# Dokumushikun/jittor-clip-fewshot

Measured on NVIDIA B200. Metric: images/sec (ViT-B/32 LoRA + MTA N=64 + LP++), higher is better.
Workload: dtype fp16

## Files before the change

### jittor-clip-fewshot_b200/csrc/gemm.cu

```cuda
#include <cstdio>
#include <mutex>
#include <unordered_map>
#include <cudaTypedefs.h>

#include "kernels.h"
#include "ptx.cuh"

namespace jcb {

namespace {

constexpr int BLOCK_M = 128;
constexpr int BLOCK_K = 64;
constexpr int UMMA_K = 16;
#ifndef JCB_GELU_WARPS
#define JCB_GELU_WARPS 4
#endif
__host__ __device__ constexpr int epi_warps_of(int epi) {
  return (epi == EPI_BIAS_GELU_BF16 || epi == EPI_LNFOLD_GELU_BF16) ? JCB_GELU_WARPS : 4;
}

#ifndef JCB_GELU_GROUP
#define JCB_GELU_GROUP 2
#endif
#ifndef JCB_GROUP
#define JCB_GROUP 2
#endif
#ifndef JCB_SMEM_KB
#define JCB_SMEM_KB 200
#endif
__host__ __device__ constexpr int group_of(int epi) { return (epi == EPI_BIAS_GELU_BF16 || epi == EPI_LNFOLD_GELU_BF16) ? JCB_GELU_GROUP : JCB_GROUP; }
__host__ __device__ constexpr bool is_lnprep(int epi) { return epi == EPI_RESID_LNPREP_SHORT || epi == EPI_RESID_LNPREP_LONG; }
__host__ __device__ constexpr bool is_lnfold(int epi) { return epi == EPI_LNFOLD_BF16 || epi == EPI_LNFOLD_GELU_BF16; }
__host__ __device__ constexpr bool out_is_bf16(int epi) { return epi == EPI_BIAS_BF16 || epi == EPI_BIAS_GELU_BF16 || is_lnfold(epi); }
#ifndef JCB_LNS_NB
#define JCB_LNS_NB 5
#endif
#ifndef JCB_LNS_D
#define JCB_LNS_D 3
#endif
#ifndef JCB_LNS_NH
#define JCB_LNS_NH 2
#endif
__host__ __device__ constexpr int lnprep_nb(int epi) { return epi == EPI_RESID_LNPREP_SHORT ? JCB_LNS_NB : 2; }
__host__ __device__ constexpr int lnprep_d(int epi) { return epi == EPI_RESID_LNPREP_SHORT ? JCB_LNS_D : 1; }
__host__ __device__ constexpr int lnprep_nh(int epi) { return epi == EPI_RESID_LNPREP_SHORT ? JCB_LNS_NH : 1; }

constexpr int CTAS = 2;

template <int BN, int EPI>
struct TileCfg {
  static constexpr int EPI_WARPS = epi_warps_of(EPI);
  static constexpr int NUM_THREADS = 64 + 32 * EPI_WARPS;
  static constexpr int HALVES = EPI_WARPS / 4;
  static constexpr int CW = BN / HALVES;
  static constexpr int GROUP = group_of(EPI) / HALVES;
  static constexpr int WARP_STAGING = (is_lnprep(EPI) ? lnprep_nb(EPI) + lnprep_nh(EPI) : GROUP) * 4096;
  static constexpr int STAGING_BYTES = EPI_WARPS * WARP_STAGING;
  static constexpr int SMEM_TOTAL = is_lnprep(EPI) ? 220 * 1024 : JCB_SMEM_KB * 1024;
  static constexpr int VEC_FLOATS = (is_lnfold(EPI) ? 2 : 1) * CW;
  static constexpr int BAR_BYTES = 512;
  static constexpr int B_ROWS = BN / CTAS;
  static constexpr int A_BYTES = BLOCK_M * BLOCK_K * 2;
  static constexpr int B_BYTES = B_ROWS * BLOCK_K * 2;
  static constexpr int STAGE_BYTES = A_BYTES + B_BYTES;
  static constexpr int STAGES = (SMEM_TOTAL - STAGING_BYTES) / STAGE_BYTES;
  static constexpr int TMEM_COLS = 2 * BN;
  static constexpr int SMEM_BYTES = STAGES * STAGE_BYTES + STAGING_BYTES + EPI_WARPS * VEC_FLOATS * 4 + BAR_BYTES + 1024;
};

struct GemmDev {
  int M, N, K;
  int K2;
  const float* bias;
  void* out;
  long long ldo;
  int* status;
  float* stats;
  int stats_slots;
  const float* colsum;
  const float* stats_in;
  const float* shift_in;
  float* shift_out;
  long long stats_in_stride;
  uint32_t idesc;
  const int* slot_of_view;
  int slot_rows;
  uint32_t slot_live;
};

__device__ __forceinline__ uint32_t tile_slot_mask(const GemmDev& p, int m_blk, int tile_m) {
  const int r0 = m_blk * tile_m;
  const int r1 = min(r0 + tile_m, p.M) - 1;
  uint32_t mask = 0;
  for (int v = r0 / p.slot_rows; v <= r1 / p.slot_rows; ++v) mask |= 1u << __ldg(p.slot_of_view + v);
  return mask & p.slot_live;
}

template <int BN, int EPI, bool F16, bool SLOTS>
__global__ void __cluster_dims__(2, 1, 1) __launch_bounds__(64 + 32 * epi_warps_of(EPI), 1)
gemm_tcgen05_2cta_kernel(const __grid_constant__ CUtensorMap tmA, const __grid_constant__ CUtensorMap tmB,
                         const __grid_constant__ CUtensorMap tmOut, const __grid_constant__ CUtensorMap tmOut2,
                         const __grid_constant__ CUtensorMap tmA2, const __grid_constant__ CUtensorMap tmB2,
                         const GemmDev p) {
  using Cfg = TileCfg<BN, EPI>;
  constexpr int STAGES = Cfg::STAGES;
  constexpr int GROUP = Cfg::GROUP;
  constexpr int WARP_STAGING = Cfg::WARP_STAGING;
  constexpr int STAGING_BYTES = Cfg::STAGING_BYTES;
  constexpr int EPI_WARPS = Cfg::EPI_WARPS;
  constexpr int CW = Cfg::CW;
  extern __shared__ uint8_t smem_raw[];
  const uint32_t raw_addr = smem_u32(smem_raw);
  uint8_t* smem = smem_raw + ((1024u - (raw_addr & 1023u)) & 1023u);
  uint8_t* ring = smem;
  uint8_t* staging = smem + STAGES * Cfg::STAGE_BYTES;
  float* s_bias_all = reinterpret_cast<float*>(staging + STAGING_BYTES);
  uint64_t* bars = reinterpret_cast<uint64_t*>(staging + STAGING_BYTES + EPI_WARPS * Cfg::VEC_FLOATS * 4);
  uint64_t* full_bar = bars;
  uint64_t* empty_bar = bars + STAGES;
  uint64_t* tmem_full_bar = bars + 2 * STAGES;
  uint64_t* tmem_empty_bar = bars + 2 * STAGES + 2;
  uint32_t* tmem_ptr_smem = reinterpret_cast<uint32_t*>(bars + 2 * STAGES + 4);
  uint64_t* load_bar = bars + 2 * STAGES + 5;

  const int warp_idx = __shfl_sync(0xffffffffu, static_cast<int>(threadIdx.x >> 5), 0);
  const int lane = threadIdx.x & 31;
  const uint32_t cta_rank = cluster_ctarank();
  const bool leader = cta_rank == 0;

  const int unit = static_cast<int>(blockIdx.x >> 1);
  const int num_units = static_cast<int>(gridDim.x >> 1);
  constexpr int TILE_M = BLOCK_M * CTAS;
  const int m_tiles = (p.M + TILE_M - 1) / TILE_M;
  const int n_tiles = p.N / BN;
  const int num_tiles = m_tiles * n_tiles;
  const int num_kb1 = p.K / BLOCK_K;
  const int num_kb = num_kb1 + p.K2 / BLOCK_K;
  constexpr uint32_t N_BLOCKS_MASK = (1u << (BN / 64)) - 1u;
  auto slot_kb_mask = [&](int m_blk) -> uint32_t { return (SLOTS && p.K2 > 0) ? tile_slot_mask(p, m_blk, TILE_M) : 0u; };
  auto slot_skip = [&](int m_blk, int n_blk) -> bool {
    return SLOTS && p.K2 == 0 && ((tile_slot_mask(p, m_blk, TILE_M) >> (n_blk * (BN / 64))) & N_BLOCKS_MASK) == 0;
  };

  if (threadIdx.x == 0) {
    tma_prefetch_desc(&tmA);
    tma_prefetch_desc(&tmB);
    if (p.K2 > 0) {
      tma_prefetch_desc(&tmA2);
      tma_prefetch_desc(&tmB2);
    }
    tma_prefetch_desc(&tmOut);
    if (is_lnprep(EPI)) {
      tma_prefetch_desc(&tmOut2);
      for (int i = 0; i < EPI_WARPS * 8; ++i) mbar_init(&load_bar[i], 1);
    }
    for (int s = 0; s < STAGES; ++s) {
      mbar_init(&full_bar[s], 1);
      mbar_init(&empty_bar[s], 1);
    }
    for (int s = 0; s < 2; ++s) {
      mbar_init(&tmem_full_bar[s], 1);
      mbar_init(&tmem_empty_bar[s], EPI_WARPS * CTAS);
    }
    fence_mbar_init();
    fence_proxy_async_smem();
  }
  if (warp_idx == 1) {
    tmem_alloc_pair(tmem_ptr_smem, Cfg::TMEM_COLS);
    tmem_relinquish_pair();
  }
  tc_fence_before();
  cluster_sync_all();
  tc_fence_after();
  const uint32_t tmem_base = *reinterpret_cast<volatile uint32_t*>(tmem_ptr_smem);
  griddep_wait();

  if (warp_idx == 0) {
    if (elect_one()) {
      int stage = 0;
      uint32_t phase = 0;
      bool ok = true;
      for (int tile = unit; tile < num_tiles && ok; tile += num_units) {
        const int m_blk = tile / n_tiles, n_blk = tile % n_tiles;
        if (slot_skip(m_blk, n_blk)) continue;
        const int m0 = m_blk * TILE_M + static_cast<int>(cta_rank) * BLOCK_M;
        const int n0 = n_blk * BN + static_cast<int>(cta_rank) * Cfg::B_ROWS;
        uint32_t kb2_rest = slot_kb_mask(m_blk);
        const int tile_kb = SLOTS && p.K2 > 0 ? num_kb1 + __popc(kb2_rest) : num_kb;
        for (int kb = 0; kb < tile_kb; ++kb) {
          if (!mbar_wait(&empty_bar[stage], phase ^ 1u, p.status, JCB_DEV_TIMEOUT_PRODUCER)) { ok = false; break; }
          uint8_t* sa = ring + stage * Cfg::STAGE_BYTES;
          uint8_t* sb = sa + Cfg::A_BYTES;
          const bool second = kb >= num_kb1;
          const CUtensorMap* ta = second ? &tmA2 : &tmA;
          const CUtensorMap* tb = second ? &tmB2 : &tmB;
          int k0 = (second ? kb - num_kb1 : kb) * BLOCK_K;
          if (SLOTS && second) {
            k0 = (__ffs(static_cast<int>(kb2_rest)) - 1) * BLOCK_K;
            kb2_rest &= kb2_rest - 1u;
          }
          if (leader) mbar_arrive_expect_tx(&full_bar[stage], 2 * Cfg::STAGE_BYTES);
          tma_load_2d_pair(sa, ta, &full_bar[stage], k0, m0);
          tma_load_2d_pair(sb, tb, &full_bar[stage], k0, n0);
          if (++stage == STAGES) { stage = 0; phase ^= 1u; }
        }
      }
    }
  } else if (warp_idx == 1) {
    if (leader && elect_one()) {
      const uint32_t idesc = p.idesc;
      int stage = 0;
      uint32_t phase = 0;
      int it = 0;
      bool ok = true;
      for (int tile = unit; tile < num_tiles && ok; tile += num_units, ++it) {
        if (slot_skip(tile / n_tiles, tile % n_tiles)) { --it; continue; }
        const int as = it & 1;
        const uint32_t aphase = (it >> 1) & 1;
        if (!mbar_wait(&tmem_empty_bar[as], aphase ^ 1u, p.status, JCB_DEV_TIMEOUT_MMA)) { ok = false; break; }
        tc_fence_after();
        const uint32_t tmem_d = tmem_base + static_cast<uint32_t>(as * BN);
        const int tile_kb = SLOTS && p.K2 > 0 ? num_kb1 + __popc(slot_kb_mask(tile / n_tiles)) : num_kb;
        for (int kb = 0; kb < tile_kb; ++kb) {
          if (!mbar_wait(&full_bar[stage], phase, p.status, JCB_DEV_TIMEOUT_MMA)) { ok = false; break; }
          tc_fence_after();
          const uint32_t sa = smem_u32(ring + stage * Cfg::STAGE_BYTES);
          const uint64_t da = umma_desc_sw128(sa);
          const uint64_t db = umma_desc_sw128(sa + Cfg::A_BYTES);
#pragma unroll
          for (int k = 0; k < BLOCK_K / UMMA_K; ++k) {
            umma_bf16_pair(tmem_d, da + static_cast<uint64_t>(2 * k), db + static_cast<uint64_t>(2 * k), idesc,
                           (kb | k) != 0 ? 1u : 0u);
          }
          umma_commit_pair(&empty_bar[stage]);
          if (++stage == STAGES) { stage = 0; phase ^= 1u; }
        }
        if (ok) umma_commit_pair(&tmem_full_bar[as]);
      }
    }
  } else {
    const int q = warp_idx & 3;
    const int ew = warp_idx - 2;
    const int col0 = (ew >> 2) * CW;
    float* s_bias = s_bias_all + ew * Cfg::VEC_FLOATS;
    float* s_csum = s_bias + CW;
    uint64_t* my_lbar = load_bar + ew * 8;
    uint32_t lphase = 0;
    const uint32_t empty_addr0 = smem_u32(&tmem_empty_bar[0]) & PEER_BIT_MASK;
    int it = 0;
    bool ok = true;
    for (int tile = unit; tile < num_tiles && ok; tile += num_units, ++it) {
      const int m_blk = tile / n_tiles, n_blk = tile % n_tiles;
      if (slot_skip(m_blk, n_blk)) { --it; continue; }
      const int as = it & 1;
      const uint32_t aphase = (it >> 1) & 1;
      __syncwarp();
      for (int i = lane; i < CW; i += 32) {
        s_bias[i] = p.bias ? __ldg(p.bias + n_blk * BN + col0 + i) : 0.0f;
        if (is_lnfold(EPI)) s_csum[i] = __ldg(p.colsum + n_blk * BN + col0 + i);
      }
      __syncwarp();
      const int row0e = m_blk * TILE_M + static_cast<int>(cta_rank) * BLOCK_M + q * 32;
      float shift = 0.f;
      if (is_lnprep(EPI)) {
        if (p.shift_in != nullptr && row0e + lane < p.M) {
          const long long r = static_cast<long long>(row0e + lane) * p.stats_in_stride;
          const float2* st = reinterpret_cast<const float2*>(p.stats_in) + r * p.stats_slots;
          float su = 0.f;
          for (int i = 0; i < p.stats_slots; ++i) su += __ldg(st + i).x;
          shift = __ldg(p.shift_in + r) + su / static_cast<float>(p.N);
        }
        if (lane == 0) {
          bulk_wait_read<0>();
#pragma unroll
          for (int d = 0; d < lnprep_d(EPI); ++d) {
            mbar_arrive_expect_tx(&my_lbar[d], 4096);
            tma_load_2d(staging + ew * WARP_STAGING + d * 4096, &tmOut, &my_lbar[d], n_blk * BN + d * 32, row0e);
          }
        }
        __syncwarp();
      }

      ok = mbar_wait(&tmem_full_bar[as], aphase, p.status, JCB_DEV_TIMEOUT_EPILOGUE);
      ok = __all_sync(0xffffffffu, ok);
      if (!ok) break;
      tc_fence_after();

      const int row0 = m_blk * TILE_M + static_cast<int>(cta_rank) * BLOCK_M + q * 32;
      const uint32_t taddr = tmem_base + (static_cast<uint32_t>(q * 32) << 16) + static_cast<uint32_t>(as * BN + col0);
      if (is_lnprep(EPI)) {
        constexpr int NB = lnprep_nb(EPI), D = lnprep_d(EPI), NH = lnprep_nh(EPI);
        constexpr int NCH = BN / 32;
        uint8_t* my_stage = staging + ew * WARP_STAGING;
        uint8_t* my_half = my_stage + NB * 4096;
        uint32_t v[2][32];
        tmem_ld_32x32b_x32(taddr, v[0]);
        float rs = 0.f, rq = 0.f;
#pragma unroll
        for (int c = 0; c < NCH; ++c) {
          uint32_t(&cur)[32] = v[c & 1];
          constexpr int WAITN = NB - D - 1;
          if (c >= 1) {
            if (lane == 0) bulk_wait_read<WAITN>();
            __syncwarp();
          }
          if (c + D < NCH && lane == 0) {
            const int nb = (c + D) % NB;
            mbar_arrive_expect_tx(&my_lbar[nb], 4096);
            tma_load_2d(my_stage + nb * 4096, &tmOut, &my_lbar[nb], n_blk * BN + (c + D) * 32, row0);
          }
          float bb[32];
#pragma unroll
          for (int j = 0; j < 8; ++j) {
            const float4 b4 = *reinterpret_cast<const float4*>(s_bias + c * 32 + 4 * j);
            bb[4 * j] = b4.x; bb[4 * j + 1] = b4.y; bb[4 * j + 2] = b4.z; bb[4 * j + 3] = b4.w;
          }
          tmem_ld_wait();
          if (c + 1 < NCH) {
            tmem_ld_32x32b_x32(taddr + static_cast<uint32_t>((c + 1) * 32), v[(c + 1) & 1]);
          } else {
            tc_fence_before();
            __syncwarp();
            if (lane == 0) mbar_arrive_cluster(empty_addr0 + static_cast<uint32_t>(as * 8));
          }
          const int b = c % NB;
          ok = mbar_wait(&my_lbar[b], (lphase >> b) & 1u, p.status, JCB_DEV_TIMEOUT_EPILOGUE);
          lphase ^= 1u << b;
          uint8_t* rowp = my_stage + b * 4096 + lane * 128;
          uint8_t* halfp = my_half + ((c >> 1) % NH) * 4096 + lane * 128;
#pragma unroll
          for (int jj = 0; jj < 4; ++jj) {
            float f[8];
#pragma unroll
            for (int h = 0; h < 2; ++h) {
              const int j = 2 * jj + h;
              float4* piece = reinterpret_cast<float4*>(rowp + ((j ^ (lane & 7)) << 4));
              float4 o = *piece;
              o.x += __uint_as_float(cur[4 * j + 0]) + bb[4 * j + 0];
              o.y += __uint_as_float(cur[4 * j + 1]) + bb[4 * j + 1];
              o.z += __uint_as_float(cur[4 * j + 2]) + bb[4 * j + 2];
              o.w += __uint_as_float(cur[4 * j + 3]) + bb[4 * j + 3];
              *piece = o;
              f[4 * h + 0] = o.x; f[4 * h + 1] = o.y; f[4 * h + 2] = o.z; f[4 * h + 3] = o.w;
            }
#pragma unroll
            for (int e = 0; e < 8; ++e) { f[e] -= shift; rs += f[e]; rq = fmaf(f[e], f[e], rq); }
            uint4 hb;
            hb.x = pack_h2<F16>(f[0], f[1]); hb.y = pack_h2<F16>(f[2], f[3]);
            hb.z = pack_h2<F16>(f[4], f[5]); hb.w = pack_h2<F16>(f[6], f[7]);
            const int hp = (c & 1) * 4 + jj;
            *reinterpret_cast<uint4*>(halfp + ((hp ^ (lane & 7)) << 4)) = hb;
          }
          fence_proxy_async_smem();
          __syncwarp();
          if (lane == 0) {
            tma_store_2d(&tmOut, my_stage + b * 4096, n_blk * BN + c * 32, row0);
            if (c & 1) tma_store_2d(&tmOut2, my_half + ((c >> 1) % NH) * 4096, n_blk * BN + (c - 1) * 32, row0);
            bulk_commit();
          }
        }
        ok = __all_sync(0xffffffffu, ok);
        if (row0 + lane < p.M) {
          *reinterpret_cast<float2*>(p.stats + (static_cast<long long>(row0 + lane) * p.stats_slots + n_blk) * 2) =
              make_float2(rs, rq);
          if (n_blk == 0 && p.shift_out != nullptr) p.shift_out[row0 + lane] = shift;
        }
      } else {
        constexpr bool OUT_BF16 = out_is_bf16(EPI);
        constexpr bool FOLD = is_lnfold(EPI);
        constexpr bool GELU = EPI == EPI_BIAS_GELU_BF16 || EPI == EPI_LNFOLD_GELU_BF16;
        constexpr int CHUNK_COLS = OUT_BF16 ? 64 : 32;
        constexpr int NCH = CW / CHUNK_COLS;
        uint8_t* my_stage = staging + ew * WARP_STAGING;
        float ln_r = 1.f, ln_nmr = 0.f;
        if (FOLD) {
          float su = 0.f, sq = 0.f;
          if (row0 + lane < p.M) {
            const float2* st = reinterpret_cast<const float2*>(p.stats) + static_cast<long long>(row0 + lane) * p.stats_slots;
            for (int i = 0; i < p.stats_slots; ++i) { const float2 t2 = __ldg(st + i); su += t2.x; sq += t2.y; }
          }
          const float inv_k = 1.0f / static_cast<float>(p.K);
          const float mean = su * inv_k;
          const float var = fmaxf(fmaf(sq, inv_k, -mean * mean), 0.f);
          ln_r = 1.0f / sqrtf(var + 1e-5f);
          ln_nmr = -mean * ln_r;
        }
        int row_slot = -1;
        if (SLOTS && p.K2 == 0 && row0 + lane < p.M) row_slot = __ldg(p.slot_of_view + (row0 + lane) / p.slot_rows);
        const int blk0 = (n_blk * BN + col0) / 64;
        (void)row_slot; (void)blk0;
        const uint64_t r2 = f2_pack(ln_r, ln_r), nmr2 = f2_pack(ln_nmr, ln_nmr);
        const uint64_t k05 = f2_pack(0.5f, 0.5f), k851 = f2_pack(0.851f, 0.851f);
        (void)r2; (void)nmr2; (void)k05; (void)k851;
        uint32_t v[2][CHUNK_COLS];
        auto load_chunk = [&](int c, uint32_t (&dst)[CHUNK_COLS]) {
          tmem_ld_32x32b_x32(taddr + static_cast<uint32_t>(c * CHUNK_COLS), *reinterpret_cast<uint32_t(*)[32]>(&dst[0]));
          if (OUT_BF16)
            tmem_ld_32x32b_x32(taddr + static_cast<uint32_t>(c * CHUNK_COLS + 32),
                               *reinterpret_cast<uint32_t(*)[32]>(&dst[CHUNK_COLS - 32]));
        };
        load_chunk(0, v[0]);
#pragma unroll
        for (int c = 0; c < NCH; ++c) {
          uint32_t(&cur)[CHUNK_COLS] = v[c & 1];
          uint64_t bb2[CHUNK_COLS / 2];
#pragma unroll
          for (int j = 0; j < CHUNK_COLS / 4; ++j) {
            const float4 b4 = *reinterpret_cast<const float4*>(s_bias + c * CHUNK_COLS + 4 * j);
            bb2[2 * j] = f2_pack(b4.x, b4.y);
            bb2[2 * j + 1] = f2_pack(b4.z, b4.w);
            if (FOLD) {
              const float4 s4 = *reinterpret_cast<const float4*>(s_csum + c * CHUNK_COLS + 4 * j);
              bb2[2 * j] = f2_fma(nmr2, f2_pack(s4.x, s4.y), bb2[2 * j]);
              bb2[2 * j + 1] = f2_fma(nmr2, f2_pack(s4.z, s4.w), bb2[2 * j + 1]);
            }
          }
          if (c % GROUP == 0) {
            if (lane == 0) bulk_wait_read<0>();
            __syncwarp();
          }
          tmem_ld_wait();
          if (c + 1 < NCH) {
            load_chunk(c + 1, v[(c + 1) & 1]);
          } else {
            tc_fence_before();
            __syncwarp();
            if (lane == 0) mbar_arrive_cluster(empty_addr0 + static_cast<uint32_t>(as * 8));
          }
          uint8_t* rowp = my_stage + (c % GROUP) * 4096 + lane * 128;
#pragma unroll
          for (int j = 0; j < 8; ++j) {
            uint4 o;
            if (OUT_BF16) {
              float f[8];
#pragma unroll
              for (int e = 0; e < 4; ++e) {
                const uint64_t a2 = f2_pack(__uint_as_float(cur[8 * j + 2 * e]), __uint_as_float(cur[8 * j + 2 * e + 1]));
                uint64_t x2 = FOLD ? f2_fma(a2, r2, bb2[4 * j + e]) : f2_add(a2, bb2[4 * j + e]);
                if (GELU) {
                  const uint64_t h2 = f2_mul(x2, k05);
                  float t0, t1;
                  f2_unpack(f2_mul(x2, k851), t0, t1);
                  x2 = f2_fma(h2, f2_pack(tanh_approx(t0), tanh_approx(t1)), h2);
                }
                f2_unpack(x2, f[2 * e], f[2 * e + 1]);
              }
              o.x = pack_h2<F16>(f[0], f[1]); o.y = pack_h2<F16>(f[2], f[3]);
              o.z = pack_h2<F16>(f[4], f[5]); o.w = pack_h2<F16>(f[6], f[7]);
              if (SLOTS && p.K2 == 0 && row_slot != blk0 + c) o = make_uint4(0u, 0u, 0u, 0u);
            } else {
              float f0, f1, f2, f3;
              f2_unpack(f2_add(f2_pack(__uint_as_float(cur[4 * j + 0]), __uint_as_float(cur[4 * j + 1])), bb2[2 * j]), f0, f1);
              f2_unpack(f2_add(f2_pack(__uint_as_float(cur[4 * j + 2]), __uint_as_float(cur[4 * j + 3])), bb2[2 * j + 1]), f2, f3);
              o.x = __float_as_uint(f0); o.y = __float_as_uint(f1); o.z = __float_as_uint(f2); o.w = __float_as_uint(f3);
            }
            *reinterpret_cast<uint4*>(rowp + ((j ^ (lane & 7)) << 4)) = o;
          }
          if (c % GROUP == GROUP - 1 || c == NCH - 1) {
            fence_proxy_async_smem();
            __syncwarp();
            if (lane == 0) {
              constexpr int G0 = 0;
#pragma unroll
              for (int g = c - (c % GROUP); g <= c; ++g) {
                const uint8_t* src = my_stage + (g % GROUP) * 4096;
                if (EPI == EPI_BIAS_RESID_F32) tma_reduce_add_2d(&tmOut, src, n_blk * BN + col0 + g * CHUNK_COLS, row0);
                else tma_store_2d(&tmOut, src, n_blk * BN + col0 + g * CHUNK_COLS, row0);
              }
              (void)G0;
              bulk_commit();
            }
          }
        }
      }
    }
    if (lane == 0) bulk_wait<0>();
  }

  tc_fence_before();
  cluster_sync_all();
  if (warp_idx == 1) {
    tc_fence_after();
    tmem_dealloc_pair(tmem_base, Cfg::TMEM_COLS);
  }
}

PFN_cuTensorMapEncodeTiled_v12000 g_encode_tiled = nullptr;
char g_driver_err[256] = {0};

struct TmapKey {
  const void* base; uint64_t rows, cols, ld; uint32_t box_rows, box_cols; int dtype;
  bool operator==(const TmapKey& o) const {
    return base == o.base && rows == o.rows && cols == o.cols && ld == o.ld && box_rows == o.box_rows &&
           box_cols == o.box_cols && dtype == o.dtype;
  }
};
struct TmapKeyHash {
  size_t operator()(const TmapKey& k) const {
    uint64_t h = reinterpret_cast<uintptr_t>(k.base) * 0x9E3779B97F4A7C15ull;
    h ^= (k.rows + 0x9E3779B97F4A7C15ull + (h << 6) + (h >> 2));
    h ^= (k.cols * 1315423911ull + k.ld * 2654435761ull + (h << 6) + (h >> 2));
    h ^= (static_cast<uint64_t>(k.box_rows) << 40) ^ (static_cast<uint64_t>(k.box_cols) << 20) ^ static_cast<uint64_t>(k.dtype);
    return static_cast<size_t>(h);
  }
};
std::mutex g_tmap_mu;
std::unordered_map<TmapKey, CUtensorMap, TmapKeyHash> g_tmap_cache;
uint64_t g_tmap_hits = 0, g_tmap_misses = 0;

bool make_tmap_2d(CUtensorMap* tm, int dtype, const void* base, uint64_t rows, uint64_t cols, uint64_t ld_elems,
                  uint32_t box_rows, uint32_t box_cols) {
  const TmapKey key{base, rows, cols, ld_elems, box_rows, box_cols, dtype};
  {
    std::lock_guard<std::mutex> lock(g_tmap_mu);
    auto it = g_tmap_cache.find(key);
    if (it != g_tmap_cache.end()) { *tm = it->second; ++g_tmap_hits; return true; }
  }
  const uint64_t esz = dtype == TM_F32 ? 4 : 2;
  cuuint64_t gdim[2] = {cols, rows};
  cuuint64_t gstride[1] = {ld_elems * esz};
  cuuint32_t box[2] = {box_cols, box_rows};
  cuuint32_t estr[2] = {1, 1};
  const CUtensorMapDataType dt = dtype == TM_F32 ? CU_TENSOR_MAP_DATA_TYPE_FLOAT32
                                 : dtype == TM_F16 ? CU_TENSOR_MAP_DATA_TYPE_FLOAT16 : CU_TENSOR_MAP_DATA_TYPE_BFLOAT16;
  CUresult r = g_encode_tiled(tm, dt, 2, const_cast<void*>(base), gdim, gstride, box, estr, CU_TENSOR_MAP_INTERLEAVE_NONE,
                              CU_TENSOR_MAP_SWIZZLE_128B, CU_TENSOR_MAP_L2_PROMOTION_L2_256B,
                              CU_TENSOR_MAP_FLOAT_OOB_FILL_NONE);
  if (r != CUDA_SUCCESS) return false;
  std::lock_guard<std::mutex> lock(g_tmap_mu);
  if (g_tmap_cache.size() >= 8192) g_tmap_cache.clear();
  g_tmap_cache.emplace(key, *tm);
  ++g_tmap_misses;
  return true;
}

template <int BN, int EPI, bool F16, bool SLOTS = false>
cudaError_t launch_cfg(const GemmArgs& a, int* dev_status, int num_sms, cudaStream_t stream) {
  using Cfg = TileCfg<BN, EPI>;
  const int op_dt = a.f16 ? TM_F16 : TM_BF16;
  CUtensorMap tmA, tmB, tmOut;
  if (!make_tmap_2d(&tmA, op_dt, a.A, a.M, a.K, a.lda, BLOCK_M, BLOCK_K)) return cudaErrorInvalidValue;
  if (!make_tmap_2d(&tmB, op_dt, a.B, a.N, a.K, a.ldb, Cfg::B_ROWS, BLOCK_K)) return cudaErrorInvalidValue;
  constexpr bool OUT_BF16 = out_is_bf16(EPI);
  CUtensorMap tmOut2;
  if (!make_tmap_2d(&tmOut, OUT_BF16 ? op_dt : TM_F32, a.out, a.M, a.N, a.ldo, 32, OUT_BF16 ? 64 : 32)) return cudaErrorInvalidValue;
  tmOut2 = tmOut;
  if (is_lnprep(EPI)) {
    if (!a.out2 || !a.stats || a.stats_slots < a.N / BN) return cudaErrorInvalidValue;
    if ((a.shift_in != nullptr) != (a.stats_in != nullptr) || a.stats_in == a.stats) return cudaErrorInvalidValue;
    if (!make_tmap_2d(&tmOut2, op_dt, a.out2, a.M, a.N, a.ldo2, 32, 64)) return cudaErrorInvalidValue;
  }
  if (is_lnfold(EPI) && (!a.stats || !a.colsum || a.stats_slots < 1)) return cudaErrorInvalidValue;
  CUtensorMap tmA2 = tmA, tmB2 = tmB;
  if (a.K2 > 0) {
    if (!make_tmap_2d(&tmA2, op_dt, a.A2, a.M, a.K2, a.lda2, BLOCK_M, BLOCK_K)) return cudaErrorInvalidValue;
    if (!make_tmap_2d(&tmB2, op_dt, a.B2, a.N, a.K2, a.ldb2, Cfg::B_ROWS, BLOCK_K)) return cudaErrorInvalidValue;
  }
  auto kern = gemm_tcgen05_2cta_kernel<BN, EPI, F16, SLOTS>;
  {
// ... 91 lines not shown
```

### jittor-clip-fewshot_b200/csrc/ptx.cuh

```cuda
#pragma once
#include <cstdint>
#include <cuda.h>
#include <cuda_bf16.h>
#include <cuda_fp16.h>
#include <cuda_runtime.h>

namespace jcb {

enum : int {
  JCB_DEV_OK = 0,
  JCB_DEV_TIMEOUT_PRODUCER = 101,
  JCB_DEV_TIMEOUT_MMA = 102,
  JCB_DEV_TIMEOUT_EPILOGUE = 103,
  JCB_DEV_SMEM_ALIGN = 104,
};

__device__ __forceinline__ uint32_t smem_u32(const void* p) {
  return static_cast<uint32_t>(__cvta_generic_to_shared(p));
}
__device__ __forceinline__ uint64_t globaltimer_ns() {
  uint64_t t;
  asm volatile("mov.u64 %0, %%globaltimer;" : "=l"(t));
  return t;
}
__device__ __forceinline__ bool elect_one() {
  uint32_t pred;
  asm volatile(
      "{\n\t.reg .pred p;\n\t"
      "elect.sync _|p, 0xffffffff;\n\t"
      "selp.u32 %0, 1, 0, p;\n\t}"
      : "=r"(pred));
  return pred != 0;
}

__device__ __forceinline__ void mbar_init(uint64_t* bar, uint32_t count) {
  asm volatile("mbarrier.init.shared::cta.b64 [%0], %1;" ::"r"(smem_u32(bar)), "r"(count) : "memory");
}
__device__ __forceinline__ void fence_mbar_init() {
  asm volatile("fence.mbarrier_init.release.cluster;" ::: "memory");
}
__device__ __forceinline__ void fence_proxy_async_smem() {
  asm volatile("fence.proxy.async.shared::cta;" ::: "memory");
}
__device__ __forceinline__ void mbar_arrive_expect_tx(uint64_t* bar, uint32_t bytes) {
  asm volatile("mbarrier.arrive.expect_tx.shared::cta.b64 _, [%0], %1;" ::"r"(smem_u32(bar)), "r"(bytes)
               : "memory");
}
__device__ __forceinline__ void mbar_arrive(uint64_t* bar) {
  asm volatile("mbarrier.arrive.shared::cta.b64 _, [%0];" ::"r"(smem_u32(bar)) : "memory");
}
__device__ __forceinline__ bool mbar_try_wait(uint64_t* bar, uint32_t parity) {
  uint32_t ok;
  asm volatile(
      "{\n\t.reg .pred p;\n\t"
      "mbarrier.try_wait.parity.shared::cta.b64 p, [%1], %2;\n\t"
      "selp.u32 %0, 1, 0, p;\n\t}"
      : "=r"(ok)
      : "r"(smem_u32(bar)), "r"(parity)
      : "memory");
  return ok != 0;
}
#ifndef JCB_MBAR_TIMEOUT_NS
#define JCB_MBAR_TIMEOUT_NS 2000000000ull
#endif
__device__ __forceinline__ bool mbar_wait(uint64_t* bar, uint32_t parity, int* status, int code) {
  if (mbar_try_wait(bar, parity)) return true;
  const uint64_t t0 = globaltimer_ns();
  uint32_t spins = 0;
  while (!mbar_try_wait(bar, parity)) {
    if (((++spins) & 255u) == 0u) {
      if (*reinterpret_cast<volatile int*>(status) != 0) return false;
      if (globaltimer_ns() - t0 > JCB_MBAR_TIMEOUT_NS) {
        atomicCAS(status, 0, code);
        return false;
      }
    }
  }
  return true;
}

__device__ __forceinline__ void tma_prefetch_desc(const CUtensorMap* tm) {
  asm volatile("prefetch.tensormap [%0];" ::"l"(reinterpret_cast<uint64_t>(tm)) : "memory");
}
__device__ __forceinline__ void tma_load_2d(void* smem_dst, const CUtensorMap* tm, uint64_t* bar, int c0,
                                            int c1) {
  asm volatile(
      "cp.async.bulk.tensor.2d.shared::cluster.global.mbarrier::complete_tx::bytes [%0], [%1, {%3, %4}], [%2];"
      ::"r"(smem_u32(smem_dst)), "l"(reinterpret_cast<uint64_t>(tm)), "r"(smem_u32(bar)), "r"(c0), "r"(c1)
      : "memory");
}


__device__ __forceinline__ void tma_store_2d(const CUtensorMap* tm, const void* smem_src, int c0, int c1) {
  asm volatile("cp.async.bulk.tensor.2d.global.shared::cta.bulk_group [%0, {%2, %3}], [%1];" ::"l"(
                   reinterpret_cast<uint64_t>(tm)),
               "r"(smem_u32(smem_src)), "r"(c0), "r"(c1)
               : "memory");
}
__device__ __forceinline__ void tma_reduce_add_2d(const CUtensorMap* tm, const void* smem_src, int c0, int c1) {
  asm volatile("cp.reduce.async.bulk.tensor.2d.global.shared::cta.add.bulk_group [%0, {%2, %3}], [%1];" ::"l"(
                   reinterpret_cast<uint64_t>(tm)),
               "r"(smem_u32(smem_src)), "r"(c0), "r"(c1)
               : "memory");
}
__device__ __forceinline__ void bulk_commit() { asm volatile("cp.async.bulk.commit_group;" ::: "memory"); }
template <int N>
__device__ __forceinline__ void bulk_wait_read() {
  asm volatile("cp.async.bulk.wait_group.read %0;" ::"n"(N) : "memory");
}
template <int N>
__device__ __forceinline__ void bulk_wait() {
  asm volatile("cp.async.bulk.wait_group %0;" ::"n"(N) : "memory");
}
__device__ __forceinline__ float tanh_approx(float x) {
  float y;
  asm("tanh.approx.f32 %0, %1;" : "=f"(y) : "f"(x));
  return y;
}

__device__ __forceinline__ void tmem_alloc(uint32_t* dst_smem, uint32_t ncols) {
  asm volatile("tcgen05.alloc.cta_group::1.sync.aligned.shared::cta.b32 [%0], %1;" ::"r"(smem_u32(dst_smem)),
               "r"(ncols)
               : "memory");
}
__device__ __forceinline__ void tmem_relinquish() {
  asm volatile("tcgen05.relinquish_alloc_permit.cta_group::1.sync.aligned;" ::: "memory");
}
__device__ __forceinline__ void tmem_dealloc(uint32_t taddr, uint32_t ncols) {
  asm volatile("tcgen05.dealloc.cta_group::1.sync.aligned.b32 %0, %1;" ::"r"(taddr), "r"(ncols) : "memory");
}
__device__ __forceinline__ void tc_fence_before() {
  asm volatile("tcgen05.fence::before_thread_sync;" ::: "memory");
}
__device__ __forceinline__ void tc_fence_after() {
  asm volatile("tcgen05.fence::after_thread_sync;" ::: "memory");
}
__device__ __forceinline__ void umma_commit(uint64_t* bar) {
  asm volatile("tcgen05.commit.cta_group::1.mbarrier::arrive::one.shared::cluster.b64 [%0];" ::"r"(
                   smem_u32(bar))
               : "memory");
}
__device__ __forceinline__ uint64_t umma_desc_sw128(uint32_t smem_addr) {
  uint64_t d = 0;
  d |= static_cast<uint64_t>((smem_addr & 0x3FFFFu) >> 4);
  d |= static_cast<uint64_t>(1) << 16;
  d |= static_cast<uint64_t>(1024 >> 4) << 32;
  d |= static_cast<uint64_t>(1) << 46;
  d |= static_cast<uint64_t>(2) << 61;
  return d;
}
__host__ __device__ constexpr uint32_t umma_idesc_bf16_f32(int m, int n) {
  return (1u << 4) | (1u << 7) | (1u << 10) | (static_cast<uint32_t>(n >> 3) << 17) |
         (static_cast<uint32_t>(m >> 4) << 24);
}
__host__ __device__ constexpr uint32_t umma_idesc_f32acc(bool f16, int m, int n, bool b_mn_major = false) {
  return (1u << 4) | (f16 ? 0u : ((1u << 7) | (1u << 10))) | (b_mn_major ? (1u << 16) : 0u) |
         (static_cast<uint32_t>(n >> 3) << 17) | (static_cast<uint32_t>(m >> 4) << 24);
}
__device__ __forceinline__ void umma_bf16(uint32_t tmem_d, uint64_t desc_a, uint64_t desc_b, uint32_t idesc,
                                          uint32_t accumulate) {
  asm volatile(
      "{\n\t.reg .pred p;\n\t"
      "setp.ne.b32 p, %4, 0;\n\t"
      "tcgen05.mma.cta_group::1.kind::f16 [%0], %1, %2, %3, p;\n\t}"
      ::"r"(tmem_d), "l"(desc_a), "l"(desc_b), "r"(idesc), "r"(accumulate)
      : "memory");
}
__device__ __forceinline__ void tmem_ld_32x32b_x32(uint32_t taddr, uint32_t (&v)[32]) {
  asm volatile(
      "tcgen05.ld.sync.aligned.32x32b.x32.b32 "
      "{%0, %1, %2, %3, %4, %5, %6, %7, %8, %9, %10, %11, %12, %13, %14, %15, "
      "%16, %17, %18, %19, %20, %21, %22, %23, %24, %25, %26, %27, %28, %29, %30, %31}, [%32];"
      : "=r"(v[0]), "=r"(v[1]), "=r"(v[2]), "=r"(v[3]), "=r"(v[4]), "=r"(v[5]), "=r"(v[6]), "=r"(v[7]),
        "=r"(v[8]), "=r"(v[9]), "=r"(v[10]), "=r"(v[11]), "=r"(v[12]), "=r"(v[13]), "=r"(v[14]), "=r"(v[15]),
        "=r"(v[16]), "=r"(v[17]), "=r"(v[18]), "=r"(v[19]), "=r"(v[20]), "=r"(v[21]), "=r"(v[22]),
// ... 184 lines not shown
```

Measured before the change: 1552.

## Add dedicated TMA loader warp for residual LN-prep epilogue loads

For the short LN-prep epilogue, the kernel gains an extra warp that issues all residual-tile TMA loads into a per-warp ring of buffers. Free/full mbarriers coordinate it with the epilogue warps, which no longer issue their own loads. Bias now comes from global memory via __ldg instead of being staged in shared memory. Optional L2 evict-first cache hints are added but off by default. The goal is to take load issue and wait latency off the epilogue critical path, at the cost of an extra warp, more barriers and per-element bias loads.

```diff
diff --git a/jittor-clip-fewshot_b200/csrc/gemm.cu b/jittor-clip-fewshot_b200/csrc/gemm.cu
--- a/jittor-clip-fewshot_b200/csrc/gemm.cu
+++ b/jittor-clip-fewshot_b200/csrc/gemm.cu
@@ -36,30 +36,34 @@
 #ifndef JCB_LNS_NB
 #define JCB_LNS_NB 5
 #endif
-#ifndef JCB_LNS_D
-#define JCB_LNS_D 3
+#ifndef JCB_LNS_K
+#define JCB_LNS_K 1
 #endif
-#ifndef JCB_LNS_NH
-#define JCB_LNS_NH 2
+#ifndef JCB_LNS_HINT
+#define JCB_LNS_HINT 0
 #endif
-__host__ __device__ constexpr int lnprep_nb(int epi) { return epi == EPI_RESID_LNPREP_SHORT ? JCB_LNS_NB : 2; }
-__host__ __device__ constexpr int lnprep_d(int epi) { return epi == EPI_RESID_LNPREP_SHORT ? JCB_LNS_D : 1; }
-__host__ __device__ constexpr int lnprep_nh(int epi) { return epi == EPI_RESID_LNPREP_SHORT ? JCB_LNS_NH : 1; }
+#ifndef JCB_LNS_SMEM_KB
+#define JCB_LNS_SMEM_KB 220
+#endif
+__host__ __device__ constexpr bool has_loader(int epi) { return epi == EPI_RESID_LNPREP_SHORT; }
+__host__ __device__ constexpr int lnprep_nb(int epi) { return has_loader(epi) ? JCB_LNS_NB : 2; }
+__host__ __device__ constexpr int lnprep_nh(int epi) { return has_loader(epi) ? 2 : 1; }
+__host__ __device__ constexpr int num_threads_of(int epi) { return 64 + 32 * epi_warps_of(epi) + (has_loader(epi) ? 32 : 0); }
 
 constexpr int CTAS = 2;
 
 template <int BN, int EPI>
 struct TileCfg {
   static constexpr int EPI_WARPS = epi_warps_of(EPI);
-  static constexpr int NUM_THREADS = 64 + 32 * EPI_WARPS;
+  static constexpr int NUM_THREADS = num_threads_of(EPI);
   static constexpr int HALVES = EPI_WARPS / 4;
   static constexpr int CW = BN / HALVES;
   static constexpr int GROUP = group_of(EPI) / HALVES;
   static constexpr int WARP_STAGING = (is_lnprep(EPI) ? lnprep_nb(EPI) + lnprep_nh(EPI) : GROUP) * 4096;
   static constexpr int STAGING_BYTES = EPI_WARPS * WARP_STAGING;
-  static constexpr int SMEM_TOTAL = is_lnprep(EPI) ? 220 * 1024 : JCB_SMEM_KB * 1024;
-  static constexpr int VEC_FLOATS = (is_lnfold(EPI) ? 2 : 1) * CW;
-  static constexpr int BAR_BYTES = 512;
+  static constexpr int SMEM_TOTAL = has_loader(EPI) ? JCB_LNS_SMEM_KB * 1024 : is_lnprep(EPI) ? 220 * 1024 : JCB_SMEM_KB * 1024;
+  static constexpr int VEC_FLOATS = has_loader(EPI) ? 0 : (is_lnfold(EPI) ? 2 : 1) * CW;
+  static constexpr int BAR_BYTES = has_loader(EPI) ? 1024 : 512;
   static constexpr int B_ROWS = BN / CTAS;
   static constexpr int A_BYTES = BLOCK_M * BLOCK_K * 2;
   static constexpr int B_BYTES = B_ROWS * BLOCK_K * 2;
@@ -98,7 +102,7 @@
 }
 
 template <int BN, int EPI, bool F16, bool SLOTS>
-__global__ void __cluster_dims__(2, 1, 1) __launch_bounds__(64 + 32 * epi_warps_of(EPI), 1)
+__global__ void __cluster_dims__(2, 1, 1) __launch_bounds__(num_threads_of(EPI), 1)
 gemm_tcgen05_2cta_kernel(const __grid_constant__ CUtensorMap tmA, const __grid_constant__ CUtensorMap tmB,
                          const __grid_constant__ CUtensorMap tmOut, const __grid_constant__ CUtensorMap tmOut2,
                          const __grid_constant__ CUtensorMap tmA2, const __grid_constant__ CUtensorMap tmB2,
@@ -123,6 +127,13 @@
   uint64_t* tmem_empty_bar = bars + 2 * STAGES + 2;
   uint32_t* tmem_ptr_smem = reinterpret_cast<uint32_t*>(bars + 2 * STAGES + 4);
   uint64_t* load_bar = bars + 2 * STAGES + 5;
+  uint64_t* free_bar = load_bar + EPI_WARPS * 8;
+  constexpr bool LOADER = has_loader(EPI);
+  constexpr int NB = lnprep_nb(EPI);
+  static_assert(!LOADER || (EPI_WARPS == 4 && NB <= 8 && JCB_LNS_K >= 0 && NB > JCB_LNS_K + 1 &&
+                            JCB_LNS_K <= 2 * lnprep_nh(EPI) - 2 && (BN / 32) % (2 * lnprep_nh(EPI)) == 0),
+                "loader ring: a buffer per chunk in flight, bf16 buffers reused in the same order in every tile");
+  static_assert(Cfg::BAR_BYTES >= (2 * STAGES + 5 + (LOADER ? 2 : 1) * EPI_WARPS * 8) * 8, "barrier region");
 
   const int warp_idx = __shfl_sync(0xffffffffu, static_cast<int>(threadIdx.x >> 5), 0);
   const int lane = threadIdx.x & 31;
@@ -154,6 +165,8 @@
     if (is_lnprep(EPI)) {
       tma_prefetch_desc(&tmOut2);
       for (int i = 0; i < EPI_WARPS * 8; ++i) mbar_init(&load_bar[i], 1);
+      if (LOADER)
+        for (int i = 0; i < EPI_WARPS * 8; ++i) mbar_init(&free_bar[i], 1);
     }
     for (int s = 0; s < STAGES; ++s) {
       mbar_init(&full_bar[s], 1);
@@ -239,7 +252,7 @@
         if (ok) umma_commit_pair(&tmem_full_bar[as]);
       }
     }
-  } else {
+  } else if (warp_idx < 2 + EPI_WARPS) {
     const int q = warp_idx & 3;
     const int ew = warp_idx - 2;
     const int col0 = (ew >> 2) * CW;
@@ -247,6 +260,9 @@
     float* s_csum = s_bias + CW;
     uint64_t* my_lbar = load_bar + ew * 8;
     uint32_t lphase = 0;
+    int rbuf = 0;
+    uint32_t rphase = 0;
+    int rfree = 0, rdone = 0;
     const uint32_t empty_addr0 = smem_u32(&tmem_empty_bar[0]) & PEER_BIT_MASK;
     int it = 0;
     bool ok = true;
@@ -256,7 +272,7 @@
       const int as = it & 1;
       const uint32_t aphase = (it >> 1) & 1;
       __syncwarp();
-      for (int i = lane; i < CW; i += 32) {
+      for (int i = lane; i < (LOADER ? 0 : CW); i += 32) {
         s_bias[i] = p.bias ? __ldg(p.bias + n_blk * BN + col0 + i) : 0.0f;
         if (is_lnfold(EPI)) s_csum[i] = __ldg(p.colsum + n_blk * BN + col0 + i);
       }
@@ -271,15 +287,14 @@
           for (int i = 0; i < p.stats_slots; ++i) su += __ldg(st + i).x;
           shift = __ldg(p.shift_in + r) + su / static_cast<float>(p.N);
         }
-        if (lane == 0) {
-          bulk_wait_read<0>();
-#pragma unroll
-          for (int d = 0; d < lnprep_d(EPI); ++d) {
-            mbar_arrive_expect_tx(&my_lbar[d], 4096);
-            tma_load_2d(staging + ew * WARP_STAGING + d * 4096, &tmOut, &my_lbar[d], n_blk * BN + d * 32, row0e);
-          }
-        }
-        __syncwarp();
+        if (!LOADER) {
+          if (lane == 0) {
+            bulk_wait_read<0>();
+            mbar_arrive_expect_tx(&my_lbar[0], 4096);
+            tma_load_2d(staging + ew * WARP_STAGING, &tmOut, &my_lbar[0], n_blk * BN, row0e);
+          }
+          __syncwarp();
+        }
       }
 
       ok = mbar_wait(&tmem_full_bar[as], aphase, p.status, JCB_DEV_TIMEOUT_EPILOGUE);
@@ -290,7 +305,7 @@
       const int row0 = m_blk * TILE_M + static_cast<int>(cta_rank) * BLOCK_M + q * 32;
       const uint32_t taddr = tmem_base + (static_cast<uint32_t>(q * 32) << 16) + static_cast<uint32_t>(as * BN + col0);
       if (is_lnprep(EPI)) {
-        constexpr int NB = lnprep_nb(EPI), D = lnprep_d(EPI), NH = lnprep_nh(EPI);
+        constexpr int D = 1, NH = lnprep_nh(EPI);
         constexpr int NCH = BN / 32;
         uint8_t* my_stage = staging + ew * WARP_STAGING;
         uint8_t* my_half = my_stage + NB * 4096;
@@ -300,21 +315,38 @@
 #pragma unroll
         for (int c = 0; c < NCH; ++c) {
           uint32_t(&cur)[32] = v[c & 1];
-          constexpr int WAITN = NB - D - 1;
-          if (c >= 1) {
-            if (lane == 0) bulk_wait_read<WAITN>();
+          if (LOADER) {
+            if (lane == 0) {
+              bulk_wait_read<JCB_LNS_K>();
+              if (rdone > JCB_LNS_K) {
+                mbar_arrive(&free_bar[ew * 8 + rfree]);
+                if (++rfree == NB) rfree = 0;
+              }
+            }
             __syncwarp();
-          }
-          if (c + D < NCH && lane == 0) {
-            const int nb = (c + D) % NB;
-            mbar_arrive_expect_tx(&my_lbar[nb], 4096);
-            tma_load_2d(my_stage + nb * 4096, &tmOut, &my_lbar[nb], n_blk * BN + (c + D) * 32, row0);
+            ++rdone;
+          } else {
+            constexpr int WAITN = NB - D - 1;
+            if (c >= 1) {
+              if (lane == 0) bulk_wait_read<WAITN>();
+              __syncwarp();
+            }
+            if (c + D < NCH && lane == 0) {
+              const int nb = (c + D) % NB;
+              mbar_arrive_expect_tx(&my_lbar[nb], 4096);
+              tma_load_2d(my_stage + nb * 4096, &tmOut, &my_lbar[nb], n_blk * BN + (c + D) * 32, row0);
+            }
           }
           float bb[32];
 #pragma unroll
           for (int j = 0; j < 8; ++j) {
-            const float4 b4 = *reinterpret_cast<const float4*>(s_bias + c * 32 + 4 * j);
-            bb[4 * j] = b4.x; bb[4 * j + 1] = b4.y; bb[4 * j + 2] = b4.z; bb[4 * j + 3] = b4.w;
+            if (LOADER) {
+#pragma unroll
+              for (int e = 0; e < 4; ++e) bb[4 * j + e] = p.bias ? __ldg(p.bias + n_blk * BN + c * 32 + 4 * j + e) : 0.0f;
+            } else {
+              const float4 b4 = *reinterpret_cast<const float4*>(s_bias + c * 32 + 4 * j);
+              bb[4 * j] = b4.x; bb[4 * j + 1] = b4.y; bb[4 * j + 2] = b4.z; bb[4 * j + 3] = b4.w;
+            }
           }
           tmem_ld_wait();
           if (c + 1 < NCH) {
@@ -324,9 +356,13 @@
             __syncwarp();
             if (lane == 0) mbar_arrive_cluster(empty_addr0 + static_cast<uint32_t>(as * 8));
           }
-          const int b = c % NB;
-          ok = mbar_wait(&my_lbar[b], (lphase >> b) & 1u, p.status, JCB_DEV_TIMEOUT_EPILOGUE);
-          lphase ^= 1u << b;
+          const int b = LOADER ? rbuf : c % NB;
+          ok = mbar_wait(&my_lbar[b], LOADER ? rphase : (lphase >> b) & 1u, p.status, JCB_DEV_TIMEOUT_EPILOGUE);
+          if (LOADER) {
+            if (++rbuf == NB) { rbuf = 0; rphase ^= 1u; }
+          } else {
+            lphase ^= 1u << b;
+          }
           uint8_t* rowp = my_stage + b * 4096 + lane * 128;
           uint8_t* halfp = my_half + ((c >> 1) % NH) * 4096 + lane * 128;
 #pragma unroll
@@ -355,7 +391,8 @@
           fence_proxy_async_smem();
           __syncwarp();
           if (lane == 0) {
-            tma_store_2d(&tmOut, my_stage + b * 4096, n_blk * BN + c * 32, row0);
+            if (LOADER && JCB_LNS_HINT) tma_store_2d_hint(&tmOut, my_stage + b * 4096, n_blk * BN + c * 32, row0, l2_evict_first_policy());
+            else tma_store_2d(&tmOut, my_stage + b * 4096, n_blk * BN + c * 32, row0);
             if (c & 1) tma_store_2d(&tmOut2, my_half + ((c >> 1) % NH) * 4096, n_blk * BN + (c - 1) * 32, row0);
             bulk_commit();
           }
@@ -476,6 +513,29 @@
       }
     }
     if (lane == 0) bulk_wait<0>();
+  } else if (LOADER) {
+    if (elect_one()) {
+      int buf = 0;
+      uint32_t phase = 0;
+      bool ok = true;
+      for (int tile = unit; tile < num_tiles && ok; tile += num_units) {
+        const int m_blk = tile / n_tiles, n_blk = tile % n_tiles;
+        const int row0c = m_blk * TILE_M + static_cast<int>(cta_rank) * BLOCK_M;
+        for (int c = 0; c < BN / 32 && ok; ++c) {
+          for (int ew = 0; ew < EPI_WARPS; ++ew) {
+            if (!mbar_wait(&free_bar[ew * 8 + buf], phase ^ 1u, p.status, JCB_DEV_TIMEOUT_PRODUCER)) { ok = false; break; }
+            mbar_arrive_expect_tx(&load_bar[ew * 8 + buf], 4096);
+            if (JCB_LNS_HINT)
+              tma_load_2d_hint(staging + ew * WARP_STAGING + buf * 4096, &tmOut, &load_bar[ew * 8 + buf], n_blk * BN + c * 32,
+                               row0c + ((ew + 2) & 3) * 32, l2_evict_first_policy());
+            else
+              tma_load_2d(staging + ew * WARP_STAGING + buf * 4096, &tmOut, &load_bar[ew * 8 + buf], n_blk * BN + c * 32,
+                          row0c + ((ew + 2) & 3) * 32);
+          }
+          if (++buf == NB) { buf = 0; phase ^= 1u; }
+        }
+      }
+    }
   }
 
   tc_fence_before();
diff --git a/jittor-clip-fewshot_b200/csrc/ptx.cuh b/jittor-clip-fewshot_b200/csrc/ptx.cuh
--- a/jittor-clip-fewshot_b200/csrc/ptx.cuh
+++ b/jittor-clip-fewshot_b200/csrc/ptx.cuh
@@ -89,8 +89,25 @@
       ::"r"(smem_u32(smem_dst)), "l"(reinterpret_cast<uint64_t>(tm)), "r"(smem_u32(bar)), "r"(c0), "r"(c1)
       : "memory");
 }
-
-
+__device__ __forceinline__ uint64_t l2_evict_first_policy() {
+  uint64_t pol;
+  asm volatile("createpolicy.fractional.L2::evict_first.b64 %0, 1.0;" : "=l"(pol));
+  return pol;
+}
+__device__ __forceinline__ void tma_load_2d_hint(void* smem_dst, const CUtensorMap* tm, uint64_t* bar, int c0, int c1,
+                                                 uint64_t policy) {
+  asm volatile(
+      "cp.async.bulk.tensor.2d.shared::cluster.global.mbarrier::complete_tx::bytes.L2::cache_hint [%0], [%1, {%3, %4}], [%2], %5;"
+      ::"r"(smem_u32(smem_dst)), "l"(reinterpret_cast<uint64_t>(tm)), "r"(smem_u32(bar)), "r"(c0), "r"(c1), "l"(policy)
+      : "memory");
+}
+
+__device__ __forceinline__ void tma_store_2d_hint(const CUtensorMap* tm, const void* smem_src, int c0, int c1, uint64_t policy) {
+  asm volatile("cp.async.bulk.tensor.2d.global.shared::cta.bulk_group.L2::cache_hint [%0, {%2, %3}], [%1], %4;" ::"l"(
+                   reinterpret_cast<uint64_t>(tm)),
+               "r"(smem_u32(smem_src)), "r"(c0), "r"(c1), "l"(policy)
+               : "memory");
+}
 __device__ __forceinline__ void tma_store_2d(const CUtensorMap* tm, const void* smem_src, int c0, int c1) {
   asm volatile("cp.async.bulk.tensor.2d.global.shared::cta.bulk_group [%0, {%2, %3}], [%1];" ::"l"(
                    reinterpret_cast<uint64_t>(tm)),
```

Result: no change. 1547, median of 6 (-0.3%).

## Add dedicated residual-load producer warp for LNPREP epilogue with full/empty ring

Applied to the files above, without the earlier changes.

Moves residual tile TMA loads in the LNPREP epilogue from each epilogue warp's lane 0 into a new dedicated producer warp. The producer and consumers coordinate through per-warp full/empty mbarrier rings, so loads can run ahead across tiles instead of being prefetched only within a tile. The bias is now read directly from global memory instead of being staged in shared memory, which frees space for more pipeline stages. The cost is an extra warp per CTA and a more complex barrier protocol, with buffers released after a lagged bulk_wait_read.

```diff
diff --git a/jittor-clip-fewshot_b200/csrc/gemm.cu b/jittor-clip-fewshot_b200/csrc/gemm.cu
--- a/jittor-clip-fewshot_b200/csrc/gemm.cu
+++ b/jittor-clip-fewshot_b200/csrc/gemm.cu
@@ -34,39 +34,44 @@
 __host__ __device__ constexpr bool is_lnfold(int epi) { return epi == EPI_LNFOLD_BF16 || epi == EPI_LNFOLD_GELU_BF16; }
 __host__ __device__ constexpr bool out_is_bf16(int epi) { return epi == EPI_BIAS_BF16 || epi == EPI_BIAS_GELU_BF16 || is_lnfold(epi); }
 #ifndef JCB_LNS_NB
-#define JCB_LNS_NB 5
-#endif
-#ifndef JCB_LNS_D
-#define JCB_LNS_D 3
+#define JCB_LNS_NB 4
 #endif
 #ifndef JCB_LNS_NH
 #define JCB_LNS_NH 2
 #endif
 __host__ __device__ constexpr int lnprep_nb(int epi) { return epi == EPI_RESID_LNPREP_SHORT ? JCB_LNS_NB : 2; }
-__host__ __device__ constexpr int lnprep_d(int epi) { return epi == EPI_RESID_LNPREP_SHORT ? JCB_LNS_D : 1; }
 __host__ __device__ constexpr int lnprep_nh(int epi) { return epi == EPI_RESID_LNPREP_SHORT ? JCB_LNS_NH : 1; }
+#ifndef JCB_LNS_LAG
+#define JCB_LNS_LAG 1
+#endif
+__host__ __device__ constexpr int lnprep_lag(int epi) { return epi == EPI_RESID_LNPREP_SHORT ? JCB_LNS_LAG : 0; }
+__host__ __device__ constexpr int threads_of(int epi) { return 64 + 32 * epi_warps_of(epi) + (is_lnprep(epi) ? 32 : 0); }
 
 constexpr int CTAS = 2;
 
 template <int BN, int EPI>
 struct TileCfg {
   static constexpr int EPI_WARPS = epi_warps_of(EPI);
-  static constexpr int NUM_THREADS = 64 + 32 * EPI_WARPS;
+  static constexpr int NUM_THREADS = threads_of(EPI);
   static constexpr int HALVES = EPI_WARPS / 4;
   static constexpr int CW = BN / HALVES;
   static constexpr int GROUP = group_of(EPI) / HALVES;
   static constexpr int WARP_STAGING = (is_lnprep(EPI) ? lnprep_nb(EPI) + lnprep_nh(EPI) : GROUP) * 4096;
   static constexpr int STAGING_BYTES = EPI_WARPS * WARP_STAGING;
-  static constexpr int SMEM_TOTAL = is_lnprep(EPI) ? 220 * 1024 : JCB_SMEM_KB * 1024;
-  static constexpr int VEC_FLOATS = (is_lnfold(EPI) ? 2 : 1) * CW;
-  static constexpr int BAR_BYTES = 512;
+  static constexpr int SMEM_TOTAL = is_lnprep(EPI) ? 224 * 1024 : JCB_SMEM_KB * 1024;
+  static constexpr int VEC_FLOATS = is_lnprep(EPI) ? 0 : (is_lnfold(EPI) ? 2 : 1) * CW;
   static constexpr int B_ROWS = BN / CTAS;
   static constexpr int A_BYTES = BLOCK_M * BLOCK_K * 2;
   static constexpr int B_BYTES = B_ROWS * BLOCK_K * 2;
   static constexpr int STAGE_BYTES = A_BYTES + B_BYTES;
   static constexpr int STAGES = (SMEM_TOTAL - STAGING_BYTES) / STAGE_BYTES;
+  static constexpr int BAR_BYTES = is_lnprep(EPI) ? 8 * (2 * STAGES + 5 + 2 * EPI_WARPS * lnprep_nb(EPI)) : 512;
   static constexpr int TMEM_COLS = 2 * BN;
   static constexpr int SMEM_BYTES = STAGES * STAGE_BYTES + STAGING_BYTES + EPI_WARPS * VEC_FLOATS * 4 + BAR_BYTES + 1024;
+  static_assert(SMEM_BYTES <= 227 * 1024 && STAGES >= 2, "shared memory split");
+  static_assert(!is_lnprep(EPI) || (EPI_WARPS == 4 && lnprep_nh(EPI) >= 1 && lnprep_lag(EPI) >= 0 &&
+                                    lnprep_lag(EPI) <= 2 * lnprep_nh(EPI) - 2 && lnprep_lag(EPI) < lnprep_nb(EPI)),
+                "LNPREP ring: one warp per TMEM lane quarter, a freed buffer must precede the chunk waiting for it");
 };
 
 struct GemmDev {
@@ -98,7 +103,7 @@
 }
 
 template <int BN, int EPI, bool F16, bool SLOTS>
-__global__ void __cluster_dims__(2, 1, 1) __launch_bounds__(64 + 32 * epi_warps_of(EPI), 1)
+__global__ void __cluster_dims__(2, 1, 1) __launch_bounds__(threads_of(EPI), 1)
 gemm_tcgen05_2cta_kernel(const __grid_constant__ CUtensorMap tmA, const __grid_constant__ CUtensorMap tmB,
                          const __grid_constant__ CUtensorMap tmOut, const __grid_constant__ CUtensorMap tmOut2,
                          const __grid_constant__ CUtensorMap tmA2, const __grid_constant__ CUtensorMap tmB2,
@@ -122,7 +127,9 @@
   uint64_t* tmem_full_bar = bars + 2 * STAGES;
   uint64_t* tmem_empty_bar = bars + 2 * STAGES + 2;
   uint32_t* tmem_ptr_smem = reinterpret_cast<uint32_t*>(bars + 2 * STAGES + 4);
-  uint64_t* load_bar = bars + 2 * STAGES + 5;
+  constexpr int NB = lnprep_nb(EPI);
+  uint64_t* res_full = bars + 2 * STAGES + 5;
+  uint64_t* res_empty = res_full + EPI_WARPS * NB;
 
   const int warp_idx = __shfl_sync(0xffffffffu, static_cast<int>(threadIdx.x >> 5), 0);
   const int lane = threadIdx.x & 31;
@@ -153,7 +160,10 @@
     tma_prefetch_desc(&tmOut);
     if (is_lnprep(EPI)) {
       tma_prefetch_desc(&tmOut2);
-      for (int i = 0; i < EPI_WARPS * 8; ++i) mbar_init(&load_bar[i], 1);
+      for (int i = 0; i < EPI_WARPS * NB; ++i) {
+        mbar_init(&res_full[i], 1);
+        mbar_init(&res_empty[i], 1);
+      }
     }
     for (int s = 0; s < STAGES; ++s) {
       mbar_init(&full_bar[s], 1);
@@ -239,14 +249,31 @@
         if (ok) umma_commit_pair(&tmem_full_bar[as]);
       }
     }
+  } else if (is_lnprep(EPI) && warp_idx >= 2 + EPI_WARPS) {
+    if (elect_one()) {
+      constexpr int NCH = BN / 32;
+      int g = 0;
+      bool ok = true;
+      for (int tile = unit; tile < num_tiles && ok; tile += num_units) {
+        const int m_blk = tile / n_tiles, n_blk = tile % n_tiles;
+        if (slot_skip(m_blk, n_blk)) continue;
+        for (int c = 0; c < NCH && ok; ++c, ++g) {
+          const int b = g % NB;
+          for (int ew = 0; ew < EPI_WARPS; ++ew) {
+            if (!mbar_wait(&res_empty[ew * NB + b], ((g / NB) & 1) ^ 1u, p.status, JCB_DEV_TIMEOUT_PRODUCER)) { ok = false; break; }
+            const int row0 = m_blk * TILE_M + static_cast<int>(cta_rank) * BLOCK_M + ((ew + 2) & 3) * 32;
+            mbar_arrive_expect_tx(&res_full[ew * NB + b], 4096);
+            tma_load_2d(staging + ew * WARP_STAGING + b * 4096, &tmOut, &res_full[ew * NB + b], n_blk * BN + c * 32, row0);
+          }
+        }
+      }
+    }
   } else {
     const int q = warp_idx & 3;
     const int ew = warp_idx - 2;
     const int col0 = (ew >> 2) * CW;
     float* s_bias = s_bias_all + ew * Cfg::VEC_FLOATS;
     float* s_csum = s_bias + CW;
-    uint64_t* my_lbar = load_bar + ew * 8;
-    uint32_t lphase = 0;
     const uint32_t empty_addr0 = smem_u32(&tmem_empty_bar[0]) & PEER_BIT_MASK;
     int it = 0;
     bool ok = true;
@@ -256,7 +283,7 @@
       const int as = it & 1;
       const uint32_t aphase = (it >> 1) & 1;
       __syncwarp();
-      for (int i = lane; i < CW; i += 32) {
+      for (int i = lane; i < (is_lnprep(EPI) ? 0 : CW); i += 32) {
         s_bias[i] = p.bias ? __ldg(p.bias + n_blk * BN + col0 + i) : 0.0f;
         if (is_lnfold(EPI)) s_csum[i] = __ldg(p.colsum + n_blk * BN + col0 + i);
       }
@@ -271,15 +298,6 @@
           for (int i = 0; i < p.stats_slots; ++i) su += __ldg(st + i).x;
           shift = __ldg(p.shift_in + r) + su / static_cast<float>(p.N);
         }
-        if (lane == 0) {
-          bulk_wait_read<0>();
-#pragma unroll
-          for (int d = 0; d < lnprep_d(EPI); ++d) {
-            mbar_arrive_expect_tx(&my_lbar[d], 4096);
-            tma_load_2d(staging + ew * WARP_STAGING + d * 4096, &tmOut, &my_lbar[d], n_blk * BN + d * 32, row0e);
-          }
-        }
-        __syncwarp();
       }
 
       ok = mbar_wait(&tmem_full_bar[as], aphase, p.status, JCB_DEV_TIMEOUT_EPILOGUE);
@@ -290,7 +308,7 @@
       const int row0 = m_blk * TILE_M + static_cast<int>(cta_rank) * BLOCK_M + q * 32;
       const uint32_t taddr = tmem_base + (static_cast<uint32_t>(q * 32) << 16) + static_cast<uint32_t>(as * BN + col0);
       if (is_lnprep(EPI)) {
-        constexpr int NB = lnprep_nb(EPI), D = lnprep_d(EPI), NH = lnprep_nh(EPI);
+        constexpr int NH = lnprep_nh(EPI), LAG = lnprep_lag(EPI);
         constexpr int NCH = BN / 32;
         uint8_t* my_stage = staging + ew * WARP_STAGING;
         uint8_t* my_half = my_stage + NB * 4096;
@@ -300,20 +318,12 @@
 #pragma unroll
         for (int c = 0; c < NCH; ++c) {
           uint32_t(&cur)[32] = v[c & 1];
-          constexpr int WAITN = NB - D - 1;
-          if (c >= 1) {
-            if (lane == 0) bulk_wait_read<WAITN>();
-            __syncwarp();
-          }
-          if (c + D < NCH && lane == 0) {
-            const int nb = (c + D) % NB;
-            mbar_arrive_expect_tx(&my_lbar[nb], 4096);
-            tma_load_2d(my_stage + nb * 4096, &tmOut, &my_lbar[nb], n_blk * BN + (c + D) * 32, row0);
-          }
+          const int g = it * NCH + c;
           float bb[32];
 #pragma unroll
           for (int j = 0; j < 8; ++j) {
-            const float4 b4 = *reinterpret_cast<const float4*>(s_bias + c * 32 + 4 * j);
+            const float4 b4 = p.bias ? __ldg(reinterpret_cast<const float4*>(p.bias + n_blk * BN + c * 32) + j)
+                                     : make_float4(0.f, 0.f, 0.f, 0.f);
             bb[4 * j] = b4.x; bb[4 * j + 1] = b4.y; bb[4 * j + 2] = b4.z; bb[4 * j + 3] = b4.w;
           }
           tmem_ld_wait();
@@ -324,11 +334,11 @@
             __syncwarp();
             if (lane == 0) mbar_arrive_cluster(empty_addr0 + static_cast<uint32_t>(as * 8));
           }
-          const int b = c % NB;
-          ok = mbar_wait(&my_lbar[b], (lphase >> b) & 1u, p.status, JCB_DEV_TIMEOUT_EPILOGUE);
-          lphase ^= 1u << b;
+          const int b = g % NB;
+          ok = mbar_wait(&res_full[ew * NB + b], (g / NB) & 1, p.status, JCB_DEV_TIMEOUT_EPILOGUE) && ok;
           uint8_t* rowp = my_stage + b * 4096 + lane * 128;
-          uint8_t* halfp = my_half + ((c >> 1) % NH) * 4096 + lane * 128;
+          uint8_t* my_half_c = my_half + ((g >> 1) % NH) * 4096;
+          uint8_t* halfp = my_half_c + lane * 128;
 #pragma unroll
           for (int jj = 0; jj < 4; ++jj) {
             float f[8];
@@ -356,9 +366,12 @@
           __syncwarp();
           if (lane == 0) {
             tma_store_2d(&tmOut, my_stage + b * 4096, n_blk * BN + c * 32, row0);
-            if (c & 1) tma_store_2d(&tmOut2, my_half + ((c >> 1) % NH) * 4096, n_blk * BN + (c - 1) * 32, row0);
+            if (c & 1) tma_store_2d(&tmOut2, my_half_c, n_blk * BN + (c - 1) * 32, row0);
             bulk_commit();
-          }
+            bulk_wait_read<LAG>();
+            if (g >= LAG) mbar_arrive(&res_empty[ew * NB + (g - LAG) % NB]);
+          }
+          __syncwarp();
         }
         ok = __all_sync(0xffffffffu, ok);
         if (row0 + lane < p.M) {
```

Measured after the change: 1620 before, 1626 after (median of 6 runs). Within noise of the previous version (+0.3%).
